# LimpBunion22/VIT-FPGA

Hardware: AMD Instinct MI355X
Metric: images/sec ViT-B/16 224x224, batch 512 per GPU (higher is better)
Workload: dtype bf16; 1 GPU; vit_base 224x224x3 inference, 512 images per GPU resident in HBM, random-init weights (seed 0); global_batch=512, per_gpu_batch=512

## Files before the change

### vit-fpga_amd/csrc/gemm_epilogue.h

```cpp
#pragma once

#include "vh_common.h"

namespace vh {

#ifndef VH_EPI_ABL
#define VH_EPI_ABL 0
#endif
#ifndef VH_EPI_NT
#define VH_EPI_NT 1
#endif
template <typename V>
__device__ __forceinline__ void epi_store(V v, V* p) {
    if constexpr (VH_EPI_NT) __builtin_nontemporal_store(v, p);
    else *p = v;
}

struct EpiArgs {
    const float* bias;
    void* out;
    int M, N;
    const float* aux;
    int aux_i;
    const float* stats;
// ... 156 lines not shown
                 : "=&v"(lnst[0]), "=&v"(lnst[1]), "=&v"(lnst[2]), "=&v"(lnst[3]), "=&v"(lnst[4]), "=&v"(lnst[5]), "=&v"(lnst[6]), "=&v"(lnst[7]) : "v"(lr));
    asm volatile("" : "+v"(bv[0]), "+v"(bv[1]), "+v"(bv[2]), "+v"(bv[3]), "+v"(cv[0]), "+v"(cv[1]), "+v"(cv[2]), "+v"(cv[3]));
}

template <typename T, int EPI, int MI, int NI, int SMI = MI, bool MFULL = false, bool OTILED = false>
__device__ __forceinline__ void gemm_epilogue_staged(const f32x4 (&acc)[MI][NI], const EpiArgs& e, int m_w, int n_w,
                                                     int lane, char* sw, int prio_grp = -1, bool cpre = false) {
    static_assert(NI == 4, "staged epilogue assumes a 64-column wave tile");
    static_assert(MI % SMI == 0 && SMI % 2 == 0, "slice must divide the wave tile");
    using elem = typename T::elem;
    const int M = e.M, N = e.N;
    const int frow = lane & 15, fq = lane >> 4;
    f32x4 bv[NI], cv[NI];
    float2 lnst[epi_is_lnfold(EPI) ? MI : 1];
    auto consts_from_global = [&]() {
#pragma unroll
        for (int ni = 0; ni < NI; ++ni) {
            bv[ni] = *(const f32x4*)(e.bias + n_w + ni * 16 + fq * 4);
            if constexpr (epi_is_lnfold(EPI)) cv[ni] = *(const f32x4*)(e.aux + n_w + ni * 16 + fq * 4);
            else cv[ni] = f32x4{0.f, 0.f, 0.f, 0.f};
        }
        if constexpr (epi_is_lnfold(EPI)) {
#pragma unroll
            for (int mi = 0; mi < MI; ++mi) {
                int m = m_w + mi * 16 + frow;
                if constexpr (!MFULL) m = m < M ? m : M - 1;
                lnst[mi] = *(const float2*)(e.stats + 2 * (int64_t)m);
            }
        }
    };
    if constexpr (epi_is_lnfold(EPI) && MI == 8) {
        if (cpre) epi_consts_from_lds(sw, frow, fq, bv, cv, lnst);
        else consts_from_global();
    } else {
        consts_from_global();
    }

    if constexpr (epi_is_16bit(EPI) && (VH_EPI_ABL & 64)) {
#pragma unroll
        for (int mi = 0; mi < MI; ++mi)
#pragma unroll
            for (int ni = 0; ni < NI; ++ni) asm volatile("" :: "v"(acc[mi][ni]));
    } else if constexpr (epi_is_16bit(EPI) && epi_has_gelu(EPI) && MFULL && OTILED) {
        char* const obase = (char*)e.out + ((int64_t)(m_w >> 4) * (N >> 3) + (n_w >> 3) + (fq & 1) * 2 + (fq >> 1)) * 256 + frow * 16;
#pragma unroll
        for (int mi = 0; mi < MI; ++mi) {
            if constexpr (VH_EPI_PRIO == 1) {
                if (prio_grp >= 0 && (mi & 1) == 0) {
                    if (((mi >> 1) + prio_grp) & 1) __builtin_amdgcn_s_setprio(1);
                    else __builtin_amdgcn_s_setprio(0);
                }
            }
            float rstd = 0.f, mr = 0.f;
            if constexpr (epi_is_lnfold(EPI)) { rstd = lnst[mi].y; mr = lnst[mi].x * lnst[mi].y; }
#pragma unroll
            for (int j = 0; j < NI / 2; ++j) {
                const f32x4 v0 = epi_value16<EPI, T>(acc[mi][2 * j], bv[2 * j], cv[2 * j], mr, rstd);
                const f32x4 v1 = epi_value16<EPI, T>(acc[mi][2 * j + 1], bv[2 * j + 1], cv[2 * j + 1], mr, rstd);
                const u32x2 p0 = __builtin_bit_cast(u32x2, pack4<T>(v0[0], v0[1], v0[2], v0[3]));
                const u32x2 p1 = __builtin_bit_cast(u32x2, pack4<T>(v1[0], v1[1], v1[2], v1[3]));
                const auto sx = __builtin_amdgcn_permlane16_swap(p0[0], p1[0], false, false);
                const auto sy = __builtin_amdgcn_permlane16_swap(p0[1], p1[1], false, false);
                epi_store(u32x4{sx[0], sy[0], sx[1], sy[1]}, (u32x4*)(obase + (int64_t)mi * (N >> 3) * 256 + j * 1024));
            }
        }
        if constexpr (VH_EPI_PRIO == 1) { if (prio_grp >= 0) __builtin_amdgcn_s_setprio(0); }
// ... 365 lines not shown
```

### vit-fpga_amd/csrc/kernels_gemm5.hip

```cpp
#include <cstdlib>
#include <type_traits>

#include "gemm_epilogue.h"
#include "vh_kernels.h"

#ifndef VH_PP_SMI
#define VH_PP_SMI 2
#endif

namespace vh {

#ifndef VH_MAIN_ABL
#define VH_MAIN_ABL 0
#endif
#ifndef VH_PP_CPRE
#define VH_PP_CPRE 1
#endif
constexpr int kAblHalf = (VH_MAIN_ABL & 64) ? 1 : 0;
constexpr int kWPieces = kAblHalf ? 2 : 4;
#ifdef VH_DIAG_STAMPS
#ifndef VH_DIAG_KT
#define VH_DIAG_KT -1
#endif
#ifndef VH_DIAG_REC_IT
// ... 17 lines not shown
    return ((unsigned long long)xcc << 32) | hw;
}
#define VH_STAMP(i, expr) do { __builtin_amdgcn_sched_barrier(0); st_[i] = (expr); __builtin_amdgcn_sched_barrier(0); } while (0)
#define VH_PSTAMP(i) do { if (pst_) { __builtin_amdgcn_sched_barrier(0); const unsigned long long t_ = diag_ct(); \
    if (lane == 0) pst_[i] = t_; __builtin_amdgcn_sched_barrier(0); } } while (0)
#else
#define VH_PSTAMP(i) do { } while (0)
#define VH_STAMP_PARAM
#define VH_STAMP(i, expr) do { } while (0)
#endif

template <int EPI, bool F8>
__host__ __device__ constexpr bool pp_uses_cpre() {
    return VH_PP_CPRE && epi_is_lnfold(EPI) && !(F8 && EPI == VH_EPI_LNFOLD_GELU);
}

template <int N>
__device__ __forceinline__ void pp_wait_vmcnt() {
    asm volatile("s_waitcnt vmcnt(%0)" ::"n"(N) : "memory");
}
__device__ __forceinline__ void pp_barrier() {
    __builtin_amdgcn_sched_barrier(0);
#if VH_MAIN_ABL & 16
    return;
#endif
    __builtin_amdgcn_s_barrier();
    __builtin_amdgcn_sched_barrier(0);
}
__device__ __forceinline__ int xcd_remap(int bid, int n) {
    const int xcd = bid & 7, qd = n >> 3, rm = n & 7;
    return (xcd < rm ? xcd * (qd + 1) : rm * (qd + 1) + (xcd - rm) * qd) + (bid >> 3);
}

template <typename T, int EPI, bool PERSIST, bool F8 = false, int AST = 2, bool OT = false, bool AT = false>
__global__ void __launch_bounds__(512, 2)
gemm_nt_pp_kernel(const void* __restrict__ Av, const void* __restrict__ Wv,
                  const float* __restrict__ bias, void* __restrict__ outp, int M, int N, int K,
                  const float* __restrict__ aux, int aux_i, int tiles_m, int tiles_n, const float* __restrict__ stats,
                  void* __restrict__ out16, float* __restrict__ partials, int tile0, int sn,
                  const float* __restrict__ wscale, int64_t prow VH_STAMP_PARAM) {
    using vec8 = typename T::vec8;
#ifdef VH_DIAG_STAMPS
    unsigned long long st_[8] = {0, 0, 0, 0, 0, 0, 0, 0};
    int it_ = 0;
    constexpr int rec_it_ = PERSIST ? VH_DIAG_REC_IT : 0;
#define first_tile_ (it_ == rec_it_)
#endif
    constexpr int BM = 256, BN = 256;
    constexpr int KT_BYTES = 128;
    static_assert(!(OT || AT) || PERSIST, "tiled layouts: persistent form only");
    constexpr int KT_STEP = AT ? 2048 : KT_BYTES;
    constexpr int STAGE_BYTES = 65536, W_OFF = 32768;
    static_assert(AST == 2 || (AST == 3 && !PERSIST), "three A stages: one tile per workgroup only");
    const char* const A = (const char*)Av;
    const char* const W = (const char*)Wv;
    const int64_t row_bytes = (int64_t)K * (F8 ? 1 : 2);
    constexpr int MI = 8, NI = 4;

    extern __shared__ __attribute__((aligned(16))) char smem[];

    const int ntiles = tiles_m * tiles_n;
    const int stride = (int)gridDim.x;
    int t = tile0 + xcd_remap(blockIdx.x, stride);

    const int lane = threadIdx.x & 63;
    const int wave = __builtin_amdgcn_readfirstlane(threadIdx.x >> 6);
    const int grp = wave >> 2, wn = wave & 3;

    const int lr = lane >> 3, lc = (lane & 7) ^ lr;
    const int rb = (int)row_bytes;
    struct TileSrc { const char *a, *w; uint32_t oa[4], ow[4]; };
    int tile_m = 0, tile_n = 0;
    auto tile_coords = [&](int tt, int& tm, int& tn) {
        if (sn > 0) {
            const int blk = tiles_m * sn, sc = tt / blk, r = tt - sc * blk;
            const int width = tiles_n - sc * sn < sn ? tiles_n - sc * sn : sn;
            tm = r / width;
            tn = sc * sn + (r - tm * width);
        } else {
            tm = tt / tiles_n;
            tn = tt - tm * tiles_n;
        }
    };
    auto base_a = [&](int tm) { return A + (int64_t)tm * BM * row_bytes; };
    auto base_w = [&](int tn) { return W + (int64_t)tn * BN * row_bytes; };
    TileSrc cur;
    auto setup_tile = [&](int tt) {
        tile_coords(tt, tile_m, tile_n);
        cur.a = base_a(tile_m);
        cur.w = base_w(tile_n);
        const int ma = PERSIST ? 255 : M - 1 - tile_m * BM, mw = PERSIST ? 255 : N - 1 - tile_n * BN;
#pragma unroll
        for (int i = 0; i < 4; ++i) {
            const int r = grp * 128 + (i * 4 + wn) * 8 + lr;
            if constexpr (AT) cur.oa[i] = (uint32_t)((grp * 8 + ((i * 4 + wn) >> 1)) * (rb * 16) + ((i * 4 + wn) & 1) * 1024 + lane * 16);
            else
            cur.oa[i] = (uint32_t)((r < ma ? r : ma) * rb + lc * 16);
            if constexpr (!PERSIST) cur.ow[i] = (uint32_t)((r < mw ? r : mw) * rb + lc * 16);
        }
    };
    const int dma_off = grp * 16384 + wn * 1024;
    int par = 0;
    auto a_off = [&](int kt, int kt3) { return AST == 2 ? ((par + kt) & 1) * STAGE_BYTES : 2 * W_OFF + kt3 * 32768; };
    auto w_off = [&](int kt) { return AST == 2 ? ((par + kt) & 1) * STAGE_BYTES + W_OFF : (kt & 1) * W_OFF; };
    bool dma_on = true;
    auto dma4 = [&](const char* base, const uint32_t (&off)[4], char* dst, int pieces = 4) {
        if constexpr (VH_MAIN_ABL & 8) { if (!dma_on) return; }
#pragma unroll
        for (int i = 0; i < 4; ++i)
            if (i < pieces)
            __builtin_amdgcn_global_load_lds((const void __attribute__((address_space(1)))*)(base + off[i]),
                                             (void __attribute__((address_space(3)))*)(dst + i * 4096), 16, 0, 0);
    };
    auto issue_a = [&](int kt, int kt3 = 0) { dma4(cur.a + (int64_t)kt * KT_STEP, cur.oa, smem + a_off(kt, kt3) + dma_off); };
    auto issue_w = [&](int kt) { dma4(cur.w + (int64_t)kt * KT_STEP, PERSIST ? cur.oa : cur.ow, smem + w_off(kt) + dma_off, kWPieces); };

    const int frow = lane & 15, fq = lane >> 4;
    const int off0 = AT ? (F8 ? 2 * fq : fq) * 256 + frow * 16 : frow * 128 + (((F8 ? 2 * fq : fq) ^ (frow & 7)) << 4);
    const int off1 = AT ? (F8 ? 2 * fq + 1 : 4 + fq) * 256 + frow * 16 : frow * 128 + (((F8 ? 2 * fq + 1 : 4 | fq) ^ (frow & 7)) << 4);
    const int xbase = grp * 16384;
    const int wbase = wn * 8192;

    const int nk = (int)(row_bytes / KT_BYTES);
    constexpr bool cpre = pp_uses_cpre<EPI, F8>() && PERSIST && AST == 2;

    setup_tile(t);
    issue_w(0);
    issue_a(0);
    if (nk > 1) {
        issue_w(1);
        issue_a(1, 1);
    }
    if (nk > 1) pp_wait_vmcnt<4 + kWPieces>();
    else pp_wait_vmcnt<0>();
    pp_barrier();
    if constexpr (VH_MAIN_ABL & 8) dma_on = false;

    bool first = true;
    while (true) {
#ifdef VH_DIAG_STAMPS
        if (first_tile_) VH_STAMP(0, diag_rt());
#endif
        f32x4 acc[MI][NI];
#pragma unroll
        for (int mi = 0; mi < MI; ++mi)
#pragma unroll
            for (int ni = 0; ni < NI; ++ni) acc[mi][ni] = f32x4{0.f, 0.f, 0.f, 0.f};

        const int t_next = t + stride;
        const bool has_next = PERSIST && t_next < ntiles;
        int tm_n = 0, tn_n = 0;
        if (has_next) tile_coords(t_next, tm_n, tn_n);

        if (grp == 1) pp_barrier();
#ifdef VH_DIAG_STAMPS
        if (first_tile_) { VH_STAMP(1, diag_rt()); VH_STAMP(5, diag_ct()); }
#endif

        auto l0_issue = [&](int kt, int k3) {
            if (AST == 3) { if (kt + 2 < nk) issue_a(kt + 2, k3 == 0 ? 2 : k3 - 1); }
            else if (kt + 1 < nk) { if (kt >= 1 || (PERSIST && !first)) issue_a(kt + 1); }
            else if (has_next) {
                cur.a = base_a(tm_n);
                dma4(cur.a, cur.oa, smem + a_off(nk, 0) + dma_off);
            }
        };
        auto issue_consts = [&]() {
            char* const slice = smem + 2 * STAGE_BYTES + wave * 4096;
            const int m0 = tile_m * BM + grp * 128, n0 = tile_n * BN + wn * 64;
            if constexpr (F8) {
                const uint32_t la = (uint32_t)(uintptr_t)slice;
                uint32_t l4 = (uint32_t)lane * 4u;
                asm_lds_dma4(bias + n0, l4, la + 1024);
                asm_lds_dma4(aux + n0, l4, la + 1280);
                asm_lds_dma4(wscale + n0, l4, la + 1536);
                l4 *= 4u;
                asm_lds_dma16((const char*)stats + (int64_t)m0 * 8, l4, la);
                return;
            }
            __builtin_amdgcn_global_load_lds((const void __attribute__((address_space(1)))*)((const char*)stats + ((int64_t)m0 * 8 + lane * 16)),
                                             (void __attribute__((address_space(3)))*)slice, 16, 0, 0);
            __builtin_amdgcn_global_load_lds((const void __attribute__((address_space(1)))*)(bias + n0 + lane),
                                             (void __attribute__((address_space(3)))*)(slice + 1024), 4, 0, 0);
            __builtin_amdgcn_global_load_lds((const void __attribute__((address_space(1)))*)(aux + n0 + lane),
                                             (void __attribute__((address_space(3)))*)(slice + 1280), 4, 0, 0);
        };
        constexpr int kNC = F8 ? 4 : 3;
        auto l1_issue_wait = [&](int kt) {
            if (kt + 2 < nk) {
                issue_w(kt + 2);
                if (cpre && kt == 1) { issue_consts(); pp_wait_vmcnt<4 + kWPieces + kNC>(); }
                else
                pp_wait_vmcnt<4 + kWPieces>();
            } else if (has_next) {
                if (kt + 2 == nk) {
                    cur.w = base_w(tn_n);
                    dma4(cur.w, cur.oa, smem + w_off(nk) + dma_off, kWPieces);
                } else {
                    dma4(cur.w + KT_STEP, cur.oa, smem + w_off(nk + 1) + dma_off, kWPieces);
                }
                pp_wait_vmcnt<4 + kWPieces>();
            } else if (AST == 2 && kt + 1 < nk) {
                pp_wait_vmcnt<4>();
            } else {
                pp_wait_vmcnt<0>();
            }
        };
        auto c1_wait = [&](int kt) {
            if (AST == 2) {
                if (cpre && kt == 1) pp_wait_vmcnt<kWPieces + kNC>();
                else
                if (kt + 2 < nk || has_next) pp_wait_vmcnt<kWPieces>();
                else pp_wait_vmcnt<0>();
            }
        };

        if constexpr (F8) {
            i32x8 wf[NI], xf[MI / 2];
            const int unit = 0x7F7F7F7F;
            auto ld8 = [&](const char* p) {
                const u32x4 lo = *(const u32x4*)(p + off0), hi = *(const u32x4*)(p + off1);
                return i32x8{(int)lo[0], (int)lo[1], (int)lo[2], (int)lo[3], (int)hi[0], (int)hi[1], (int)hi[2], (int)hi[3]};
            };
            for (int kt = 0, k3 = 0; kt < nk; ++kt, k3 = k3 == 2 ? 0 : k3 + 1) {
                const char* sa = smem + a_off(kt, k3) + xbase;
                const char* sw = smem + w_off(kt) + wbase;
#pragma unroll
                for (int ni = 0; ni < NI; ++ni) wf[ni] = ld8(sw + ni * 2048);
#pragma unroll
                for (int mi = 0; mi < MI / 2; ++mi) xf[mi] = ld8(sa + mi * 2048);
                l0_issue(kt, k3);
                __builtin_amdgcn_s_waitcnt(0xC07F);
                pp_barrier();
                __builtin_amdgcn_s_setprio(1);
#pragma unroll
                for (int mi = 0; mi < MI / 2; ++mi)
// ... 57 lines not shown
            VH_PSTAMP(3);
            pp_barrier();
            VH_PSTAMP(4);
#pragma unroll
            for (int mi = 0; mi < MI_A; ++mi) {
                if constexpr (VH_MAIN_ABL & 2) { asm volatile("" : "=v"(xf[mi])); continue; }
                if constexpr (VH_MAIN_ABL & 4) { asm volatile("" : "+v"(xf[mi])); continue; }
                xf[mi] = *(const vec8*)(sa + mi * 2048 + off1);
            }
            l1_issue_wait(kt);
            __builtin_amdgcn_s_waitcnt(0xC07F);
            VH_PSTAMP(5);
            pp_barrier();
            VH_PSTAMP(6);
            if constexpr (!(VH_MAIN_ABL & 32)) __builtin_amdgcn_s_setprio(1);
#pragma unroll
            for (int mi = 0; mi < MI_A; ++mi)
#pragma unroll
                for (int ni = 0; ni < NI; ++ni) {
                    if constexpr (VH_MAIN_ABL & 1) asm volatile("" : "+v"(acc[mi][ni]) : "v"(wf1[ni]), "v"(xf[mi]));
                    else acc[mi][ni] = T::mfma16(wf1[ni], xf[mi], acc[mi][ni]);
                }
            __builtin_amdgcn_s_setprio(0);
            c1_wait(kt);
            VH_PSTAMP(7);
            pp_barrier();
        }
        }
        if (grp == 0) pp_barrier();
#ifdef VH_DIAG_STAMPS
        if (first_tile_) { VH_STAMP(6, diag_ct()); VH_STAMP(2, diag_rt()); }
#endif

        const int m_w = tile_m * BM + grp * 128, n_w = tile_n * BN + wn * 64;
        const bool m_full = (tile_m + 1) * BM <= M, n_full = (tile_n + 1) * BN <= N;
        char* const stage_epi = smem + (PERSIST ? 2 * STAGE_BYTES : STAGE_BYTES);
        const EpiArgs e{bias, outp, M, N, aux, aux_i, stats, out16, partials, prow};
        int lane_e = lane;
        if constexpr (PERSIST) asm volatile("" : "+v"(lane_e));
        if constexpr (F8) {
#pragma clang fp contract(off)
            const int fq_e = lane_e >> 4;
            f32x4 wsv[NI];
            if (cpre) {
                const uint32_t la = (uint32_t)(uintptr_t)(smem + 2 * STAGE_BYTES + wave * 4096) + (uint32_t)(fq_e * 16);
                static_assert(NI == 4, "64-column wave tile");
                asm volatile("ds_read_b128 %0, %4 offset:1536\n\tds_read_b128 %1, %4 offset:1600\n\tds_read_b128 %2, %4 offset:1664\n\tds_read_b128 %3, %4 offset:1728\n\t"
                             "s_waitcnt lgkmcnt(0)" : "=&v"(wsv[0]), "=&v"(wsv[1]), "=&v"(wsv[2]), "=&v"(wsv[3]) : "v"(la));
            } else {
#pragma unroll
                for (int ni = 0; ni < NI; ++ni) {
                    const int n = n_w + ni * 16 + fq_e * 4;
                    wsv[ni] = n < N ? *(const f32x4*)(wscale + n) : f32x4{0.f, 0.f, 0.f, 0.f};
                }
            }
#pragma unroll
            for (int ni = 0; ni < NI; ++ni) {
#pragma unroll
                for (int mi = 0; mi < MI; ++mi) acc[mi][ni] = acc[mi][ni] * wsv[ni];
            }
        }
        if constexpr (PERSIST) {
            constexpr int SLICE = VH_PP_SMI * 16 * 128;
            static_assert(VH_PP_SMI == 2, "staging region of the persistent form: 8 waves x 4 KiB");
            if constexpr (F8 && epi_has_gelu(EPI))
                gemm_epilogue8<EPI, MI, NI, VH_PP_SMI, true, OT>(acc, e, m_w, n_w, lane_e, true, stage_epi, wave, cpre);
            else if constexpr (F8 && (EPI == VH_EPI_RESID_LN || EPI == VH_EPI_RESID_SPLIT))
// ... 27 lines not shown
        t = t_next;
        tile_m = tm_n;
        tile_n = tn_n;
    }
}

static int gemm_super_columns(int tiles_n) {
    static const int env = [] { const int e = env_int("VH_PP_SN", -1); return e < -1 ? -1 : e; }();
    if (env >= 0) return env > 0 && env < tiles_n ? env : 0;
    if (tiles_n < 6) return 0;
    if (tiles_n % 4 == 0) return 4;
    if (tiles_n % 3 == 0) return 3;
    return 4;
}

#ifdef VH_DIAG_STAMPS
struct DiagRec { int64_t M; int N, K, epi, f8, grid, variant; };
static unsigned long long* g_diag_buf = nullptr;
static int g_diag_slots = 0, g_diag_max_wgs = 0;
static long long g_diag_count = 0;
static DiagRec g_diag_rec[1024];
static unsigned long long* diag_next(const GemmArgs& g, int epi, bool f8, int grid, int variant) {
    if (!g_diag_buf || grid > g_diag_max_wgs) return nullptr;
    const int slot = (int)(g_diag_count % g_diag_slots);
    g_diag_rec[slot] = DiagRec{g.M, g.N, g.K, epi, f8 ? 1 : 0, grid, variant};
    ++g_diag_count;
    return g_diag_buf + (size_t)slot * g_diag_max_wgs * 128;
}
#define VH_STAMP_ARG(g, epi, f8, grid, variant) , diag_next(g, epi, f8, grid, variant)
#else
#define VH_STAMP_ARG(g, epi, f8, grid, variant)
#endif

template <typename T, int EPI, bool F8, bool PERSIST, int AST, bool OT = false, bool AT = false>
static hipError_t launch_pp_one(const GemmArgs& g, int grid, int tiles_m, int tiles_n, hipStream_t s) {
    constexpr size_t lds = (AST == 3 || PERSIST) ? 163840 : 131072;
    auto k = gemm_nt_pp_kernel<T, EPI, PERSIST, F8, AST, OT, AT>;
    static LdsDone lds_done;
    if (hipError_t e = ensure_dynamic_lds((const void*)k, lds, lds_done); e != hipSuccess) return e;
    hipLaunchKernelGGL(k, dim3(grid), dim3(512), lds, s, g.a, g.w, g.bias, g.out, (int)g.M, g.N, g.K, g.aux, g.aux_i, tiles_m,
                       tiles_n, g.stats, g.out16, g.partials, PERSIST ? 0 : g.tile_begin, (g.tile_count || g.tile_begin) ? 0 : gemm_super_columns(tiles_n),
                       F8 ? (g.wscale ? g.wscale : g.aux) : (const float*)nullptr, gemm_prow(g)
                       VH_STAMP_ARG(g, EPI, F8, grid, PERSIST ? 6 : (AST == 3 ? 7 : 5)));
    return hipGetLastError();
}

template <typename T, int EPI, bool F8>
static hipError_t launch_pp(const GemmArgs& g, int mode, hipStream_t s) {
    if constexpr (EPI == VH_EPI_PATCH) { if (mode == 1) mode = 0; }
    const int tiles_m = (int)((g.M + 255) / 256), tiles_n = (g.N + 255) / 256;
    int ntiles = tiles_m * tiles_n;
    if (g.tile_count > 0) {
        if (mode == 1 || g.tile_begin < 0 || g.tile_begin + g.tile_count > ntiles) return hipErrorInvalidValue;
        ntiles = g.tile_count;
    } else if (g.tile_begin != 0) {
        return hipErrorInvalidValue;
    }
    if (mode == 2) return launch_pp_one<T, EPI, F8, false, 3>(g, ntiles, tiles_m, tiles_n, s);
    if constexpr (EPI != VH_EPI_PATCH) {
        const int full_m = (int)(g.M / 256);
        const int nk = g.K / (F8 ? 128 : 64);
        if (mode == 1 && (g.N % 256 != 0 || full_m == 0 || nk < (pp_uses_cpre<EPI, F8>() ? 4 : 2))) mode = 0;
        if (mode == 1 && full_m != tiles_m && g.variant != 6) mode = 0;
        if ((g.out_tiled || g.ab_tiled) && (mode != 1 || full_m != tiles_m)) return hipErrorInvalidValue;
        if (mode == 1) {
            const int num_cu = device_num_cu();
            if (!num_cu) return hipErrorUnknown;
            const int nfull = full_m * tiles_n;
            if constexpr (EPI == VH_EPI_LNFOLD_GELU || EPI == VH_EPI_BIAS_GELU || EPI == VH_EPI_LNFOLD || (!F8 && EPI == VH_EPI_BIAS)) {
                if (g.out_tiled) return g.ab_tiled ? hipErrorInvalidValue : launch_pp_one<T, EPI, F8, true, 2, true, false>(g, nfull < num_cu ? nfull : num_cu, full_m, tiles_n, s);
            }
            if constexpr (F8 ? EPI == VH_EPI_RESID_SPLIT : (EPI == VH_EPI_RESID_SPLIT || EPI == VH_EPI_BIAS)) {
                if (g.ab_tiled) return g.out_tiled ? hipErrorInvalidValue : launch_pp_one<T, EPI, F8, true, 2, false, true>(g, nfull < num_cu ? nfull : num_cu, full_m, tiles_n, s);
            }
            if (g.out_tiled || g.ab_tiled) return hipErrorInvalidValue;
            if (hipError_t e = launch_pp_one<T, EPI, F8, true, 2>(g, nfull < num_cu ? nfull : num_cu, full_m, tiles_n, s); e != hipSuccess) return e;
            if (full_m == tiles_m) return hipSuccess;
            GemmArgs tail = g;
            tail.tile_begin = nfull;
            tail.tile_count = tiles_n;
            return launch_pp_one<T, EPI, F8, false, 2>(tail, tiles_n, tiles_m, tiles_n, s);
        }
    }
    if (g.out_tiled || g.ab_tiled) return hipErrorInvalidValue;
    return launch_pp_one<T, EPI, F8, false, 2>(g, ntiles, tiles_m, tiles_n, s);
}

template <typename T, int EPI>
hipError_t launch_gemm_pingpong(const GemmArgs& g, int mode, hipStream_t s) {
    return launch_pp<T, EPI, false>(g, mode, s);
}

#define VH_INST(T)                                                                                     \
    template hipError_t launch_gemm_pingpong<T, VH_EPI_BIAS>(const GemmArgs&, int, hipStream_t);       \
    template hipError_t launch_gemm_pingpong<T, VH_EPI_BIAS_GELU>(const GemmArgs&, int, hipStream_t);  \
    template hipError_t launch_gemm_pingpong<T, VH_EPI_BIAS_RESID>(const GemmArgs&, int, hipStream_t); \
    template hipError_t launch_gemm_pingpong<T, VH_EPI_BIAS_F32>(const GemmArgs&, int, hipStream_t);   \
    template hipError_t launch_gemm_pingpong<T, VH_EPI_PATCH>(const GemmArgs&, int, hipStream_t);       \
    template hipError_t launch_gemm_pingpong<T, VH_EPI_LNFOLD>(const GemmArgs&, int, hipStream_t);      \
    template hipError_t launch_gemm_pingpong<T, VH_EPI_LNFOLD_GELU>(const GemmArgs&, int, hipStream_t); \
    template hipError_t launch_gemm_pingpong<T, VH_EPI_RESID_LN>(const GemmArgs&, int, hipStream_t);   \
    template hipError_t launch_gemm_pingpong<T, VH_EPI_RESID_SPLIT>(const GemmArgs&, int, hipStream_t); \
    template hipError_t launch_gemm_pingpong<T, VH_EPI_PATCH_SPLIT>(const GemmArgs&, int, hipStream_t);
VH_INST(BF16)
VH_INST(FP16)

hipError_t launch_gemm_fp8(const GemmArgs& g, hipStream_t s) {
    const int v = g.variant ? g.variant : gemm_pp_variant(g.epilogue);
    const int mode = v == 7 ? 2 : (v == 6 && !g.tile_count && !g.tile_begin ? 1 : 0);
    switch (g.epilogue) {
// ... 38 lines not shown
```

### vit-fpga_amd/csrc/vh_kernels.h

```cpp
#pragma once

#include <atomic>
#include <cstdlib>

#include "vh_common.h"

namespace vh {

struct GemmArgs {
    const void* a;
    const void* w;
    const float* bias;
    void* out;
    int64_t M;
    int N, K;
    int epilogue;
    const float* aux;
    int aux_i;
    int dtype;
    int variant;
    const float* stats = nullptr;
    void* out16 = nullptr;
    float* partials = nullptr;
    const float* wscale = nullptr;
    int tile_begin = 0, tile_count = 0;
    int64_t prow = 0;
    int out_tiled = 0, ab_tiled = 0;
};
bool gemm_tiled_applies(int64_t M, int N, int K);
hipError_t launch_cast_tiled_w(const float* w, int rows, int cols, void* w16, int dtype, hipStream_t stream);
bool gemm_tiled_applies_f8(int64_t M, int N, int K);
hipError_t launch_tile_bytes(const void* w8, int rows, int cols, void* out, hipStream_t stream);

inline int64_t gemm_prow(const GemmArgs& g) {
    if (g.epilogue != VH_EPI_PATCH_SPLIT) return g.M;
    return g.prow > 0 ? g.prow : (g.M / g.aux_i) * (int64_t)(g.aux_i + 1);
}

hipError_t launch_gemm(const GemmArgs& g, hipStream_t stream);
hipError_t launch_gemm_fp8(const GemmArgs& g, hipStream_t stream);
const char* gemm_check(const GemmArgs& g);
int gemm_pick_variant(int64_t M, int N, int epilogue);
int gemm_pp_variant(int epilogue);

hipError_t launch_layernorm(const float* x, int64_t rows, int dim, int64_t row_stride,
                            const float* gamma, const float* beta, float eps, void* out16,
                            int dtype, hipStream_t stream);
constexpr int VH_DTYPE_F32_INTERNAL = 100;
hipError_t launch_head_f32(const float* y, const float* w, const float* bias, float* out, int batch, int classes, int dim,
                           hipStream_t stream);
constexpr float kAttnQScale = 0.125f * 1.4426950408889634f;
hipError_t launch_attention(const void* qkv16, int batch, int tokens, int heads, void* out16,
                            int dtype, unsigned int* ticket, hipStream_t stream, bool ticket_zeroed = false, bool out_tiled = false,
                            int64_t in_hm_rows = 0);
bool attention_tiled_applies(int batch, int tokens, int heads);
hipError_t launch_attention_cls(const void* qkv16, int batch, int tokens, int heads, void* out16, int dtype, hipStream_t stream);
size_t attention_lds_bytes(int tokens);
constexpr int kAttnStreamMaxTokens = 4097;
hipError_t launch_attention_stream(const void* qkv16, int batch, int tokens, int heads, void* out16, int dtype, hipStream_t stream);
constexpr int kAttnHdMaxWidth = 2048;
bool attention_hd_supported(int head_dim);
hipError_t launch_attention_hd(const void* qkv16, int batch, int tokens, int heads, int head_dim, void* out16, int dtype,
                               hipStream_t stream);
inline float attention_q_scale(int head_dim) {
    return head_dim == 64 ? kAttnQScale : (float)(1.4426950408889634 / __builtin_sqrt((double)head_dim));
}
hipError_t launch_im2col(const float* in_nhwc, int batch, int image, int patch, int channels, int kpad,
                         void* out16, int dtype, hipStream_t stream);
bool patch_fused_supported(int image, int patch, int channels, int dim);
hipError_t launch_patch_fused(const float* images, int batch, int image, int patch, int channels, const void* wp16, const float* bias,
                              const float* pos, void* hi, void* lo, float* partials, int64_t prow, int dim, int dtype, hipStream_t stream);
hipError_t launch_cls_rows(float* x, const float* cls, const float* pos, int batch, int tokens,
                           int dim, hipStream_t stream);
hipError_t launch_cls_rows_split(void* hi, void* lo, float* partials, int64_t prow, const float* cls, const float* pos, int batch,
                                 int tokens, int dim, int dtype, hipStream_t stream);
hipError_t launch_cast(const float* in, void* out16, int64_t n, int dtype, hipStream_t stream);
// ... 63 lines not shown
```

### vit-fpga_amd/csrc/vithip_api.hip

```cpp
#include <dlfcn.h>

#include <chrono>
#include <condition_variable>
#include <cstdarg>
#include <cstdio>
#include <cstdlib>
#include <cstring>
#include <functional>
#include <memory>
#include <mutex>
#include <string>
#include <thread>
#include <vector>

#include "vh_kernels.h"

using namespace vh;

namespace {

thread_local std::string g_err;

int fail(std::string* ctx_err, int code, const char* fmt, ...) {
    char buf[512];
// ... 142 lines not shown
    bool ln_fold_cfg = false, split_cfg = false;
    unsigned int* guard_dev = nullptr;
    float* guard_host = nullptr;
    float guard_thresh = 0.5f;
    bool guard_auto = false, guard_tripped = false;
    char* arena = nullptr;
    unsigned int* tickets = nullptr;
    float* x = nullptr;
    void* xn16 = nullptr;
    void* qkv16 = nullptr;
    void* att16 = nullptr;
    void* h16 = nullptr;
    void* col16 = nullptr;
    float* clsn32 = nullptr;
    float* in_dev = nullptr;
    float* logits_dev = nullptr;
    int64_t last_us = 0;
    bool timed = false;
    int last_batch = 0;
    struct RingSlot {
        float *h_in = nullptr, *h_out = nullptr, *d_in = nullptr, *d_out = nullptr;
        hipEvent_t in_done = nullptr, fwd_done = nullptr, out_done = nullptr;
        int batch = 0;
    };
    std::vector<RingSlot> ring;
    hipStream_t copy_in = nullptr, copy_out = nullptr;
    int ring_batch = 0, ring_wr = 0, ring_rd = 0, ring_used = 0;
    hipStream_t tstream = nullptr;
    hipEvent_t ev_tail_a = nullptr, ev_tail_l = nullptr;
    bool tail_overlap = false;
    bool last_h_tiled = false;
    bool last_qkv_hm = false;
    int tail_splits = 0;
    int num_cu = 256;
    bool use_graph = false;
    struct GraphEntry { const float* in; float* out; int batch; hipGraph_t graph; hipGraphExec_t exec; };
    std::vector<GraphEntry> graphs;
    std::vector<int> graph_warm;
    int timing_stage = -1;
    std::vector<hipEvent_t> tev;
    size_t tev_used = 0;
    bool step_timing = false;
    std::vector<hipEvent_t> sev;
    size_t sev_used = 0;
    std::string err;
};

struct vh_filter {
    int device, height, width, kind;
    struct Slot {
        uint8_t *h_in = nullptr, *h_out = nullptr, *d_in = nullptr, *d_out = nullptr;
        hipEvent_t in_done = nullptr, k_done = nullptr, out_done = nullptr;
    };
    std::vector<Slot> slot;
    hipStream_t copy_in = nullptr, compute = nullptr, copy_out = nullptr;
    int wr = 0, rd = 0, used = 0;
    std::string err;
};

struct vh_mlp {
    int device, n_ins, n_layers, activation;
    std::vector<int> npl;
    size_t n_params = 0, n_neurons = 0;
    int widest = 0, max_vec = 0;
    hipStream_t stream = nullptr;
    float *params = nullptr, *bias = nullptr, *buf0 = nullptr, *buf1 = nullptr;
// ... 144 lines not shown
    auto mark = [&](int stage) -> int {
        if (!ev) return VH_OK;
        hipEvent_t e;
        HIPCHK(&c->err, hipEventCreate(&e));
        HIPCHK(&c->err, hipEventRecord(e, s));
        ev->push_back({stage, e});
        return VH_OK;
    };
    auto gemm = [&](const void* a, const void* w, const float* bias, void* out, int64_t Mr, int N, int K, int epi,
                    const float* aux, int aux_i, const float* wscale = nullptr) {
        GemmArgs g{a, w, bias, out, Mr, N, K, epi, aux, aux_i, dt16, 0};
        g.stats = stats_p;
        g.out16 = epi == VH_EPI_RESID_SPLIT ? xlo16 : xn16;
        g.partials = partials_p;
        if (wscale) {
            g.dtype = VH_DTYPE_FP8;
            if (epi == VH_EPI_LNFOLD || epi == VH_EPI_LNFOLD_GELU) g.wscale = wscale;
            else g.aux = wscale;
            return launch_gemm_fp8(g, s);
        }
        return launch_gemm(g, s);
    };
    auto tmark = [&](int stage) -> int {
        if (stage != c->timing_stage) return VH_OK;
        if (c->tev_used == c->tev.size()) {
            hipEvent_t e;
            HIPCHK(&c->err, hipEventCreate(&e));
            c->tev.push_back(e);
        }
        HIPCHK(&c->err, hipEventRecord(c->tev[c->tev_used++], s));
        return VH_OK;
    };
    int rc;
    if (img0 == 0) c->tail_splits = 0;
    if ((rc = mark(-1))) return rc;
    const int nl = (c->run_layers < 0 || c->run_layers > f.layers) ? f.layers : c->run_layers;
    const bool fused_patch = c->patch_fused && c->split && !c->fp8 && nl > 0 && patch_fused_supported(f.image_size, f.patch_size, f.channels, D);
    if (!fused_patch) {
        if ((rc = tmark(ST_IM2COL))) return rc;
        HIPCHK(&c->err, launch_im2col(in, batch, f.image_size, f.patch_size, f.channels, L.KPA, col16, dt16, s));
        if ((rc = tmark(ST_IM2COL))) return rc;
    }
    if ((rc = mark(ST_IM2COL))) return rc;
    if (fused_patch) {
        if ((rc = tmark(ST_PATCH))) return rc;
        HIPCHK(&c->err, launch_patch_fused(in, batch, f.image_size, f.patch_size, f.channels, c->wp16, P + L.patch_b, P + L.pos, xn16, xlo16,
                                           partials_p, rows_g, D, dt16, s));
        if ((rc = tmark(ST_PATCH))) return rc;
        if ((rc = mark(ST_PATCH))) return rc;
        HIPCHK(&c->err, launch_cls_rows_split(xn16, xlo16, partials_p, rows_g, P + L.cls, P + L.pos, batch, T, D, dt16, s));
        if ((rc = mark(ST_CLS))) return rc;
        HIPCHK(&c->err, launch_finalize_stats(partials_p, D / 64, rows_g, D, f.ln_eps, stats_p, s, rows, c->guard_dev, amax_guard));
        if ((rc = mark(ST_LNSTATS))) return rc;
    } else if (c->split && !c->fp8 && nl > 0) {
        GemmArgs g{col16, c->wp16, P + L.patch_b, xn16, (int64_t)batch * L.NP, D, L.KPA, VH_EPI_PATCH_SPLIT, P + L.pos, L.NP, dt16, 0};
        g.out16 = xlo16; g.partials = partials_p; g.prow = rows_g;
        if ((rc = tmark(ST_PATCH))) return rc;
        HIPCHK(&c->err, launch_gemm(g, s));
        if ((rc = tmark(ST_PATCH))) return rc;
        if ((rc = mark(ST_PATCH))) return rc;
        HIPCHK(&c->err, launch_cls_rows_split(xn16, xlo16, partials_p, rows_g, P + L.cls, P + L.pos, batch, T, D, dt16, s));
        if ((rc = mark(ST_CLS))) return rc;
        HIPCHK(&c->err, launch_finalize_stats(partials_p, D / 64, rows_g, D, f.ln_eps, stats_p, s, rows, c->guard_dev, amax_guard));
        if ((rc = mark(ST_LNSTATS))) return rc;
    } else {
        if ((rc = tmark(ST_PATCH))) return rc;
        HIPCHK(&c->err, gemm(col16, c->wp16, P + L.patch_b, x, (int64_t)batch * L.NP, D, L.KPA, VH_EPI_PATCH, P + L.pos, L.NP));
// ... 1097 lines not shown
            }
            std::vector<uint16_t> hi(n);
            std::vector<uint8_t> lo(n);
            HIPCHK(&c->err, hipMemcpy(hi.data(), c->xn16, n * 2, hipMemcpyDeviceToHost));
            HIPCHK(&c->err, hipMemcpy(lo.data(), c->xlo16, n, hipMemcpyDeviceToHost));
            const float inv = c->dt16 == VH_DTYPE_BF16 ? 1.f / 32.f : 1.f / 256.f;
            for (size_t i = 0; i < n; ++i) host_out[i] = f(hi[i], c->dt16) + g(lo[i]) * inv;
            return VH_OK;
        }
        HIPCHK(&c->err, hipMemcpy(host_out, c->x, n * 4, hipMemcpyDeviceToHost));
        return VH_OK;
    }
    if (what == 1) {
        const size_t n = (size_t)c->last_batch * D;
        if (n_floats != n) return fail(&c->err, VH_ERR_INVALID, "expected %zu floats", n);
        HIPCHK(&c->err, hipMemcpy(host_out, c->clsn32, n * 4, hipMemcpyDeviceToHost));
        return VH_OK;
    }
    if (what == 2) {
        if (n_floats != 1) return fail(&c->err, VH_ERR_INVALID, "expected 1 float");
        host_out[0] = (float)c->tail_splits;
        return VH_OK;
    }
    if (what == 3) {
        if (n_floats != 1) return fail(&c->err, VH_ERR_INVALID, "expected 1 float");
        host_out[0] = c->last_h_tiled ? 1.f : 0.f;
        return VH_OK;
    }
    if (what == 4) {
        if (n_floats != 1) return fail(&c->err, VH_ERR_INVALID, "expected 1 float");
        host_out[0] = c->last_qkv_hm ? 1.f : 0.f;
        return VH_OK;
    }
    return fail(&c->err, VH_ERR_INVALID, "unknown tap %d", what);
}

int vh_debug_set_layers(vh_ctx* c, int n_layers) {
    if (!c) return fail(nullptr, VH_ERR_INVALID, "null context");
    c->run_layers = n_layers;
    if (c->stream) hipStreamSynchronize(c->stream);
    drop_graphs(c);
    return VH_OK;
}

#define OPCHK(expr) do { hipError_t e_ = (expr); if (e_ != hipSuccess) return fail(nullptr, VH_ERR_HIP, "%s failed: %s", #expr, hipGetErrorString(e_)); } while (0)

int vh_op_gemm(const void* a, const void* w, const float* bias, void* out, int64_t M, int N, int K, int epi,
               const float* aux, int aux_i, int dtype, int variant, void* stream) {
    GemmArgs g{a, w, bias, out, M, N, K, epi, aux, aux_i, dtype, variant};
    if (const char* why = gemm_check(g)) return fail(nullptr, VH_ERR_INVALID, "%s", why);
    OPCHK(launch_gemm(g, (hipStream_t)stream));
    OPCHK(hipStreamSynchronize((hipStream_t)stream));
    return VH_OK;
}
int vh_op_gemm_fp8(const void* a8, const void* w8, const float* w_scale, const float* bias, void* out, int64_t M, int N, int K,
                   int epi, int variant, void* stream) {
    if (variant != 0 && variant != 5 && variant != 6 && variant != 7) return fail(nullptr, VH_ERR_INVALID, "gemm_fp8: variant must be 0, 5, 6 or 7");
    if (!a8 || !w8 || !w_scale || !bias || !out) return fail(nullptr, VH_ERR_INVALID, "gemm_fp8: null pointer");
    if (M <= 0 || N <= 0 || K <= 0 || K % 128 || N % 4) return fail(nullptr, VH_ERR_INVALID, "gemm_fp8: need K %% 128 == 0 and N %% 4 == 0");
    if (M > 0x7FFFFFFF / 2) return fail(nullptr, VH_ERR_INVALID, "gemm_fp8: M too large");
    if (epi != VH_EPI_BIAS && epi != VH_EPI_BIAS_GELU && epi != VH_EPI_BIAS_RESID && epi != VH_EPI_BIAS_F32)
        return fail(nullptr, VH_ERR_UNSUPPORTED, "gemm_fp8: epilogue %d not available", epi);
    GemmArgs g{a8, w8, bias, out, M, N, K, epi, w_scale, 0, VH_DTYPE_FP8, variant};
    OPCHK(launch_gemm_fp8(g, (hipStream_t)stream));
    OPCHK(hipStreamSynchronize((hipStream_t)stream));
    return VH_OK;
// ... 723 lines not shown
```

Before: 28820 images/s.

## Split persistent GEMM tail wave into short-M tiles to fill idle CUs

When the number of 256x256 output tiles does not divide evenly across CUs, the persistent GEMM now runs the full rounds with 256-row tiles. It then launches a second kernel whose M tile is 64, 128 or 192 rows over the leftover rows, so the last partial wave spreads across more CUs. The kernel is templated on BM, with adjusted A load pieces, wait counts, stats prefetch and epilogue constant loading for the shorter tiles. This applies only to LN-fold and residual-split epilogues with K at least 2048 by default. In exchange it adds an extra launch and uses less efficient short tiles for the tail.

```diff
diff --git a/vit-fpga_amd/csrc/gemm_epilogue.h b/vit-fpga_amd/csrc/gemm_epilogue.h
--- a/vit-fpga_amd/csrc/gemm_epilogue.h
+++ b/vit-fpga_amd/csrc/gemm_epilogue.h
@@ -212,6 +212,15 @@
     if constexpr (epi_is_lnfold(EPI) && MI == 8) {
         if (cpre) epi_consts_from_lds(sw, frow, fq, bv, cv, lnst);
         else consts_from_global();
+    } else if constexpr (epi_is_lnfold(EPI) && MI < 8) {
+        if (cpre) {
+            float2 st8[8];
+            epi_consts_from_lds(sw, frow, fq, bv, cv, st8);
+#pragma unroll
+            for (int mi = 0; mi < MI; ++mi) lnst[mi] = st8[mi];
+        } else {
+            consts_from_global();
+        }
     } else {
         consts_from_global();
     }
diff --git a/vit-fpga_amd/csrc/kernels_gemm5.hip b/vit-fpga_amd/csrc/kernels_gemm5.hip
--- a/vit-fpga_amd/csrc/kernels_gemm5.hip
+++ b/vit-fpga_amd/csrc/kernels_gemm5.hip
@@ -73,7 +73,7 @@
     return (xcd < rm ? xcd * (qd + 1) : rm * (qd + 1) + (xcd - rm) * qd) + (bid >> 3);
 }
 
-template <typename T, int EPI, bool PERSIST, bool F8 = false, int AST = 2, bool OT = false, bool AT = false>
+template <typename T, int EPI, bool PERSIST, bool F8 = false, int AST = 2, bool OT = false, bool AT = false, int BM = 256>
 __global__ void __launch_bounds__(512, 2)
 gemm_nt_pp_kernel(const void* __restrict__ Av, const void* __restrict__ Wv,
                   const float* __restrict__ bias, void* __restrict__ outp, int M, int N, int K,
@@ -87,7 +87,10 @@
     constexpr int rec_it_ = PERSIST ? VH_DIAG_REC_IT : 0;
 #define first_tile_ (it_ == rec_it_)
 #endif
-    constexpr int BM = 256, BN = 256;
+    constexpr int BN = 256;
+    static_assert(BM == 256 || (PERSIST && !F8 && AST == 2 && (BM == 64 || BM == 128 || BM == 192)), "short tiles: persistent 16-bit form");
+    constexpr int HR = BM / 2;
+    constexpr int kAPieces = BM / 64;
     constexpr int KT_BYTES = 128;
     static_assert(!(OT || AT) || PERSIST, "tiled layouts: persistent form only");
     constexpr int KT_STEP = AT ? 2048 : KT_BYTES;
@@ -96,7 +99,7 @@
     const char* const A = (const char*)Av;
     const char* const W = (const char*)Wv;
     const int64_t row_bytes = (int64_t)K * (F8 ? 1 : 2);
-    constexpr int MI = 8, NI = 4;
+    constexpr int MI = BM / 32, NI = 4;
 
     extern __shared__ __attribute__((aligned(16))) char smem[];
 
@@ -130,14 +133,18 @@
         tile_coords(tt, tile_m, tile_n);
         cur.a = base_a(tile_m);
         cur.w = base_w(tile_n);
-        const int ma = PERSIST ? 255 : M - 1 - tile_m * BM, mw = PERSIST ? 255 : N - 1 - tile_n * BN;
+        const int ma = PERSIST ? BM - 1 : M - 1 - tile_m * BM, mw = PERSIST ? 255 : N - 1 - tile_n * BN;
 #pragma unroll
         for (int i = 0; i < 4; ++i) {
-            const int r = grp * 128 + (i * 4 + wn) * 8 + lr;
-            if constexpr (AT) cur.oa[i] = (uint32_t)((grp * 8 + ((i * 4 + wn) >> 1)) * (rb * 16) + ((i * 4 + wn) & 1) * 1024 + lane * 16);
+            const int r = grp * HR + (i * 4 + wn) * 8 + lr;
+            if constexpr (AT) cur.oa[i] = (uint32_t)((grp * (HR / 16) + ((i * 4 + wn) >> 1)) * (rb * 16) + ((i * 4 + wn) & 1) * 1024 + lane * 16);
             else
             cur.oa[i] = (uint32_t)((r < ma ? r : ma) * rb + lc * 16);
             if constexpr (!PERSIST) cur.ow[i] = (uint32_t)((r < mw ? r : mw) * rb + lc * 16);
+            else if constexpr (BM != 256) {
+                if constexpr (AT) cur.ow[i] = (uint32_t)((grp * 8 + ((i * 4 + wn) >> 1)) * (rb * 16) + ((i * 4 + wn) & 1) * 1024 + lane * 16);
+                else cur.ow[i] = (uint32_t)((grp * 128 + (i * 4 + wn) * 8 + lr) * rb + lc * 16);
+            }
         }
     };
     const int dma_off = grp * 16384 + wn * 1024;
@@ -153,8 +160,9 @@
             __builtin_amdgcn_global_load_lds((const void __attribute__((address_space(1)))*)(base + off[i]),
                                              (void __attribute__((address_space(3)))*)(dst + i * 4096), 16, 0, 0);
     };
-    auto issue_a = [&](int kt, int kt3 = 0) { dma4(cur.a + (int64_t)kt * KT_STEP, cur.oa, smem + a_off(kt, kt3) + dma_off); };
-    auto issue_w = [&](int kt) { dma4(cur.w + (int64_t)kt * KT_STEP, PERSIST ? cur.oa : cur.ow, smem + w_off(kt) + dma_off, kWPieces); };
+    auto w_offs = [&]() -> const uint32_t (&)[4] { if constexpr (PERSIST && BM == 256) return cur.oa; else return cur.ow; };
+    auto issue_a = [&](int kt, int kt3 = 0) { dma4(cur.a + (int64_t)kt * KT_STEP, cur.oa, smem + a_off(kt, kt3) + dma_off, kAPieces); };
+    auto issue_w = [&](int kt) { dma4(cur.w + (int64_t)kt * KT_STEP, w_offs(), smem + w_off(kt) + dma_off, kWPieces); };
 
     const int frow = lane & 15, fq = lane >> 4;
     const int off0 = AT ? (F8 ? 2 * fq : fq) * 256 + frow * 16 : frow * 128 + (((F8 ? 2 * fq : fq) ^ (frow & 7)) << 4);
@@ -172,7 +180,7 @@
         issue_w(1);
         issue_a(1, 1);
     }
-    if (nk > 1) pp_wait_vmcnt<4 + kWPieces>();
+    if (nk > 1) pp_wait_vmcnt<kAPieces + kWPieces>();
     else pp_wait_vmcnt<0>();
     pp_barrier();
     if constexpr (VH_MAIN_ABL & 8) dma_on = false;
@@ -203,12 +211,12 @@
             else if (kt + 1 < nk) { if (kt >= 1 || (PERSIST && !first)) issue_a(kt + 1); }
             else if (has_next) {
                 cur.a = base_a(tm_n);
-                dma4(cur.a, cur.oa, smem + a_off(nk, 0) + dma_off);
+                dma4(cur.a, cur.oa, smem + a_off(nk, 0) + dma_off, kAPieces);
             }
         };
         auto issue_consts = [&]() {
             char* const slice = smem + 2 * STAGE_BYTES + wave * 4096;
-            const int m0 = tile_m * BM + grp * 128, n0 = tile_n * BN + wn * 64;
+            const int m0 = tile_m * BM + grp * HR, n0 = tile_n * BN + wn * 64;
             if constexpr (F8) {
                 const uint32_t la = (uint32_t)(uintptr_t)slice;
                 uint32_t l4 = (uint32_t)lane * 4u;
@@ -219,7 +227,8 @@
                 asm_lds_dma16((const char*)stats + (int64_t)m0 * 8, l4, la);
                 return;
             }
-            __builtin_amdgcn_global_load_lds((const void __attribute__((address_space(1)))*)((const char*)stats + ((int64_t)m0 * 8 + lane * 16)),
+            const int ls = BM == 256 ? lane : (lane < HR / 2 ? lane : HR / 2 - 1);
+            __builtin_amdgcn_global_load_lds((const void __attribute__((address_space(1)))*)((const char*)stats + ((int64_t)m0 * 8 + ls * 16)),
                                              (void __attribute__((address_space(3)))*)slice, 16, 0, 0);
             __builtin_amdgcn_global_load_lds((const void __attribute__((address_space(1)))*)(bias + n0 + lane),
                                              (void __attribute__((address_space(3)))*)(slice + 1024), 4, 0, 0);
@@ -230,19 +239,19 @@
         auto l1_issue_wait = [&](int kt) {
             if (kt + 2 < nk) {
                 issue_w(kt + 2);
-                if (cpre && kt == 1) { issue_consts(); pp_wait_vmcnt<4 + kWPieces + kNC>(); }
+                if (cpre && kt == 1) { issue_consts(); pp_wait_vmcnt<kAPieces + kWPieces + kNC>(); }
                 else
-                pp_wait_vmcnt<4 + kWPieces>();
+                pp_wait_vmcnt<kAPieces + kWPieces>();
             } else if (has_next) {
                 if (kt + 2 == nk) {
                     cur.w = base_w(tn_n);
-                    dma4(cur.w, cur.oa, smem + w_off(nk) + dma_off, kWPieces);
+                    dma4(cur.w, w_offs(), smem + w_off(nk) + dma_off, kWPieces);
                 } else {
-                    dma4(cur.w + KT_STEP, cur.oa, smem + w_off(nk + 1) + dma_off, kWPieces);
+                    dma4(cur.w + KT_STEP, w_offs(), smem + w_off(nk + 1) + dma_off, kWPieces);
                 }
-                pp_wait_vmcnt<4 + kWPieces>();
+                pp_wait_vmcnt<kAPieces + kWPieces>();
             } else if (AST == 2 && kt + 1 < nk) {
-                pp_wait_vmcnt<4>();
+                pp_wait_vmcnt<kAPieces>();
             } else {
                 pp_wait_vmcnt<0>();
             }
@@ -366,7 +375,7 @@
         if (first_tile_) { VH_STAMP(6, diag_ct()); VH_STAMP(2, diag_rt()); }
 #endif
 
-        const int m_w = tile_m * BM + grp * 128, n_w = tile_n * BN + wn * 64;
+        const int m_w = tile_m * BM + grp * HR, n_w = tile_n * BN + wn * 64;
         const bool m_full = (tile_m + 1) * BM <= M, n_full = (tile_n + 1) * BN <= N;
         char* const stage_epi = smem + (PERSIST ? 2 * STAGE_BYTES : STAGE_BYTES);
         const EpiArgs e{bias, outp, M, N, aux, aux_i, stats, out16, partials, prow};
@@ -460,10 +469,10 @@
 #define VH_STAMP_ARG(g, epi, f8, grid, variant)
 #endif
 
-template <typename T, int EPI, bool F8, bool PERSIST, int AST, bool OT = false, bool AT = false>
+template <typename T, int EPI, bool F8, bool PERSIST, int AST, bool OT = false, bool AT = false, int BM = 256>
 static hipError_t launch_pp_one(const GemmArgs& g, int grid, int tiles_m, int tiles_n, hipStream_t s) {
     constexpr size_t lds = (AST == 3 || PERSIST) ? 163840 : 131072;
-    auto k = gemm_nt_pp_kernel<T, EPI, PERSIST, F8, AST, OT, AT>;
+    auto k = gemm_nt_pp_kernel<T, EPI, PERSIST, F8, AST, OT, AT, BM>;
     static LdsDone lds_done;
     if (hipError_t e = ensure_dynamic_lds((const void*)k, lds, lds_done); e != hipSuccess) return e;
     hipLaunchKernelGGL(k, dim3(grid), dim3(512), lds, s, g.a, g.w, g.bias, g.out, (int)g.M, g.N, g.K, g.aux, g.aux_i, tiles_m,
@@ -471,6 +480,62 @@
                        F8 ? (g.wscale ? g.wscale : g.aux) : (const float*)nullptr, gemm_prow(g)
                        VH_STAMP_ARG(g, EPI, F8, grid, PERSIST ? 6 : (AST == 3 ? 7 : 5)));
     return hipGetLastError();
+}
+
+static int gemm_tail_mode() {
+    static const int m = [] { const int e = env_int("VH_GEMM_TAIL", 1); return e < 0 || e > 2 ? 1 : e; }();
+    return m;
+}
+struct TailPlan { int full_m = 0, rows = 0, R = 0; };
+static TailPlan gemm_tail_plan(int tiles_m, int tiles_n, int K, int num_cu) {
+    TailPlan p;
+    const int mode = gemm_tail_mode();
+    if (mode == 0 || (mode == 1 && K < 2048)) return p;
+    const int64_t ntiles = (int64_t)tiles_m * tiles_n;
+    const int64_t rounds = ntiles / num_cu;
+    if (rounds == 0 || ntiles % num_cu == 0) return p;
+    const int a = (int)(rounds * num_cu / tiles_n);
+    for (int R = 64; R <= 192; R += 64) {
+        for (int fm = a; fm >= a - 2 && fm >= 1; --fm) {
+            const int rows = (tiles_m - fm) * 256;
+            if (rows % R || (int64_t)(rows / R) * tiles_n > num_cu) continue;
+            p.full_m = fm; p.rows = rows; p.R = R;
+            return p;
+        }
+    }
+    return p;
+}
+static thread_local long long g_short_tails = 0;
+long long gemm_short_tails() { return g_short_tails; }
+
+template <typename T, int EPI, bool F8, bool OT, bool AT>
+static hipError_t launch_persistent(const GemmArgs& g, int full_m, int tiles_n, int num_cu, hipStream_t s) {
+    if constexpr (!F8 && (EPI == VH_EPI_LNFOLD || EPI == VH_EPI_LNFOLD_GELU || EPI == VH_EPI_RESID_SPLIT)) {
+        const TailPlan p = gemm_tail_plan(full_m, tiles_n, g.K, num_cu);
+        if (p.R) {
+            const int nf = p.full_m * tiles_n;
+            if (hipError_t e = launch_pp_one<T, EPI, F8, true, 2, OT, AT>(g, nf < num_cu ? nf : num_cu, p.full_m, tiles_n, s); e != hipSuccess) return e;
+            const int64_t row0 = (int64_t)p.full_m * 256;
+            constexpr int64_t esz = 2;
+            GemmArgs t = g;
+            t.a = (const char*)g.a + row0 * g.K * esz;
+            constexpr bool head_major = OT && !epi_has_gelu(EPI);
+            t.out = (char*)g.out + row0 * (head_major ? 64 : g.N) * esz;
+            if constexpr (epi_is_lnfold(EPI)) t.stats = g.stats + 2 * row0;
+            if constexpr (EPI == VH_EPI_RESID_SPLIT) {
+                t.out16 = (char*)g.out16 + row0 * g.N;
+                t.partials = g.partials + 2 * row0;
+            }
+            const int tm = p.rows / p.R, n = tm * tiles_n;
+            hipError_t e = p.R == 64 ? launch_pp_one<T, EPI, F8, true, 2, OT, AT, 64>(t, n, tm, tiles_n, s)
+                         : p.R == 128 ? launch_pp_one<T, EPI, F8, true, 2, OT, AT, 128>(t, n, tm, tiles_n, s)
+                                      : launch_pp_one<T, EPI, F8, true, 2, OT, AT, 192>(t, n, tm, tiles_n, s);
+            if (e == hipSuccess) ++g_short_tails;
+            return e;
+        }
+    }
+    const int nfull = full_m * tiles_n;
+    return launch_pp_one<T, EPI, F8, true, 2, OT, AT>(g, nfull < num_cu ? nfull : num_cu, full_m, tiles_n, s);
 }
 
 template <typename T, int EPI, bool F8>
@@ -496,14 +561,14 @@
             if (!num_cu) return hipErrorUnknown;
             const int nfull = full_m * tiles_n;
             if constexpr (EPI == VH_EPI_LNFOLD_GELU || EPI == VH_EPI_BIAS_GELU || EPI == VH_EPI_LNFOLD || (!F8 && EPI == VH_EPI_BIAS)) {
-                if (g.out_tiled) return g.ab_tiled ? hipErrorInvalidValue : launch_pp_one<T, EPI, F8, true, 2, true, false>(g, nfull < num_cu ? nfull : num_cu, full_m, tiles_n, s);
+                if (g.out_tiled) return g.ab_tiled ? hipErrorInvalidValue : launch_persistent<T, EPI, F8, true, false>(g, full_m, tiles_n, num_cu, s);
             }
             if constexpr (F8 ? EPI == VH_EPI_RESID_SPLIT : (EPI == VH_EPI_RESID_SPLIT || EPI == VH_EPI_BIAS)) {
-                if (g.ab_tiled) return g.out_tiled ? hipErrorInvalidValue : launch_pp_one<T, EPI, F8, true, 2, false, true>(g, nfull < num_cu ? nfull : num_cu, full_m, tiles_n, s);
+                if (g.ab_tiled) return g.out_tiled ? hipErrorInvalidValue : launch_persistent<T, EPI, F8, false, true>(g, full_m, tiles_n, num_cu, s);
             }
             if (g.out_tiled || g.ab_tiled) return hipErrorInvalidValue;
+            if (full_m == tiles_m) return launch_persistent<T, EPI, F8, false, false>(g, full_m, tiles_n, num_cu, s);
             if (hipError_t e = launch_pp_one<T, EPI, F8, true, 2>(g, nfull < num_cu ? nfull : num_cu, full_m, tiles_n, s); e != hipSuccess) return e;
-            if (full_m == tiles_m) return hipSuccess;
             GemmArgs tail = g;
             tail.tile_begin = nfull;
             tail.tile_count = tiles_n;
diff --git a/vit-fpga_amd/csrc/vh_kernels.h b/vit-fpga_amd/csrc/vh_kernels.h
--- a/vit-fpga_amd/csrc/vh_kernels.h
+++ b/vit-fpga_amd/csrc/vh_kernels.h
@@ -42,6 +42,7 @@
 const char* gemm_check(const GemmArgs& g);
 int gemm_pick_variant(int64_t M, int N, int epilogue);
 int gemm_pp_variant(int epilogue);
+long long gemm_short_tails();
 
 hipError_t launch_layernorm(const float* x, int64_t rows, int dim, int64_t row_stride,
                             const float* gamma, const float* beta, float eps, void* out16,
diff --git a/vit-fpga_amd/csrc/vithip_api.hip b/vit-fpga_amd/csrc/vithip_api.hip
--- a/vit-fpga_amd/csrc/vithip_api.hip
+++ b/vit-fpga_amd/csrc/vithip_api.hip
@@ -198,6 +198,7 @@
     bool last_h_tiled = false;
     bool last_qkv_hm = false;
     int tail_splits = 0;
+    long long short_tails0 = 0;
     int num_cu = 256;
     bool use_graph = false;
     struct GraphEntry { const float* in; float* out; int batch; hipGraph_t graph; hipGraphExec_t exec; };
@@ -408,7 +409,7 @@
         return VH_OK;
     };
     int rc;
-    if (img0 == 0) c->tail_splits = 0;
+    if (img0 == 0) { c->tail_splits = 0; c->short_tails0 = gemm_short_tails(); }
     if ((rc = mark(-1))) return rc;
     const int nl = (c->run_layers < 0 || c->run_layers > f.layers) ? f.layers : c->run_layers;
     const bool fused_patch = c->patch_fused && c->split && !c->fp8 && nl > 0 && patch_fused_supported(f.image_size, f.patch_size, f.channels, D);
@@ -1572,6 +1573,11 @@
         host_out[0] = c->last_qkv_hm ? 1.f : 0.f;
         return VH_OK;
     }
+    if (what == 5) {
+        if (n_floats != 1) return fail(&c->err, VH_ERR_INVALID, "expected 1 float");
+        host_out[0] = (float)(gemm_short_tails() - c->short_tails0);
+        return VH_OK;
+    }
     return fail(&c->err, VH_ERR_INVALID, "unknown tap %d", what);
 }
 
```

Measured after the change: 28880 images/s, median of 6. Within noise of the previous version (+0.2%).
